# minfenli/refnerf-pl

Hardware: AMD Instinct MI355X
Metric: ray-samples/s (4096 rays x 128 samples x 2 levels, Ref-NeRF Blender, eval forward) (higher is better)
Workload: dtype f16x2; 1 GPU; blender_refnerf.gin, 4096 rays x 128 samples, 2-level, Model.__call__ eval forward with compute_extras + full ray_history; rays_per_gpu=4096, total_rays=4096, samples_per_level=128, parallelism=ray-tile dp1, n_ranks_seen=1, hip_graph_replay=False

## Files before the change

### refnerf-pl_amd/csrc/refnerf_hip.hip

```cpp
#include <hip/hip_runtime.h>

#include <cmath>
#include <cstdio>
#include <cstring>
#include <cstdlib>
#include <mutex>
#include <utility>
#include <vector>

#include "refnerf_hip.h"
#include "refnerf_level_common.h"
#include "refnerf_level_f32.h"
#include "refnerf_level_bf16.h"
#include "refnerf_level_bwd_f32.h"
#include "refnerf_wgrad.h"
#include "refnerf_wgrad_bf16x3.h"
#include "refnerf_rays.h"
#include "refnerf_pack_common.h"
#include "refnerf_sq_host.h"
#include "refnerf_sq_layout.h"

namespace rn {


// ... 659 lines not shown
  if (R <= 0) return fail(REFNERF_EINVAL, "refnerf_level_forward: R must be positive%s");
  if (cfg->n_samples <= 1) return fail(REFNERF_EINVAL, "num_samples must be > 1%s");
  if (cfg->ray_shape != 0 && cfg->ray_shape != 1) return fail(REFNERF_EINVAL, "ray_shape must be 'cone' or 'cylinder'%s");
  if (cfg->n_in < 1 || cfg->n_in > 512) return fail(REFNERF_EINVAL, "n_in must be in [1,512]%s");
  if (cfg->precision != REFNERF_PREC_F32 && cfg->precision != REFNERF_PREC_BF16 && cfg->precision != REFNERF_PREC_F16 &&
      cfg->precision != REFNERF_PREC_F16X2)
    return fail(REFNERF_EINVAL, "unknown precision mode%s");
  if (cfg->raydist < REFNERF_RAYDIST_NONE || cfg->raydist > REFNERF_RAYDIST_SQUARE)
    return fail(REFNERF_EINVAL, "unknown raydist (REFNERF_RAYDIST_*)%s");
  if (cfg->dir_enc != REFNERF_DIRENC_IDE && cfg->dir_enc != REFNERF_DIRENC_POSENC)
    return fail(REFNERF_EINVAL, "unknown dir_enc (REFNERF_DIRENC_IDE / REFNERF_DIRENC_POSENC)%s");
  if (cfg->training && cfg->precision == REFNERF_PREC_F16)
    return fail(REFNERF_EUNSUPPORTED, "REFNERF_PREC_F16 is an inference mode (training levels: REFNERF_PREC_F32, REFNERF_PREC_F16X2 or REFNERF_PREC_BF16)%s");
  const bool gbasis = cfg->ipe_groups > 1;
  if (cfg->ipe_groups < 0 || cfg->ipe_groups > rn::IPE_MAX_GROUPS) return fail(REFNERF_EINVAL, "ipe_groups must be in [0,7]%s");
  if (gbasis && cfg->precision != REFNERF_PREC_F32 && cfg->precision != REFNERF_PREC_F16X2)
    return fail(REFNERF_EUNSUPPORTED, "a general IPE basis (ipe_groups > 1) runs with REFNERF_PREC_F32 or REFNERF_PREC_F16X2 (d_packed: the REFNERF_PREC_F32 image of refnerf_pack_weights_basis in both)%s");
  const bool train_bf = cfg->training && cfg->precision == REFNERF_PREC_BF16;
  if (!rays->d_origins || !rays->d_directions || !rays->d_viewdirs || !rays->d_radii || !rays->d_near || !rays->d_far)
    return fail(REFNERF_EINVAL, "refnerf_level_forward: null ray field%s");
  const int N = cfg->n_samples;
  const bool gb_split = gbasis && cfg->precision == REFNERF_PREC_F16X2;
  if (int irc = check_image(d_packed, cfg, "refnerf_level_forward")) return irc;
  const bool train_sq = cfg->training && cfg->precision == REFNERF_PREC_F16X2 && !gbasis;
  if (train_sq && !d_act)
    return fail(REFNERF_EINVAL, "a training level in REFNERF_PREC_F16X2 runs through refnerf_level_forward_train: its kernel keeps the ReLU sign words and "
                                "the bottleneck rows in the activation buffer (d_packed: the REFNERF_IMAGE_F16X2_TRAIN image)%s");
  if (cfg->wgrad_mode == REFNERF_WGRAD_F16 && !train_sq)
    return fail(REFNERF_EUNSUPPORTED, "wgrad_mode = REFNERF_WGRAD_F16 belongs to training levels in REFNERF_PREC_F16X2 on the built-in IPE basis%s");
  if (train_sq) return rnsq::forward(d_packed, cfg, rays, R, d_sdist_in, d_weights_in, out, d_act, (hipStream_t)stream);
  const bool split = cfg->precision == REFNERF_PREC_F16X2 && !gb_split;
  const bool bf = (cfg->precision == REFNERF_PREC_BF16 && !train_bf) || cfg->precision == REFNERF_PREC_F16 || split;
  int rpw = rays_per_wg(N, bf ? rn::BT : rn::T_TILE);
  bool ps_ring = false;
  if (bf && N <= rn::BF_PS_RING - rn::BT && (rpw * N) % rn::BT != 0) {
    int r = 1;
    while (r <= rn::BF_NW && (r * N) % rn::BT != 0) ++r;
    if (r <= rn::BF_NW && r * N > 640 && R / r >= 512) { rpw = r; ps_ring = true; }
  }
  auto lds_bytes = [&](int rays) -> size_t {
    const int np = bf ? rn::NPS_EVAL : rn::NPS_TRAIN, tile = bf ? rn::BT : rn::T_TILE;
    const int ps_rows = ps_ring ? rn::BF_PS_RING : rays * N;
    const size_t per_wg = sizeof(float) * (size_t)(2 * rays * (N + 1) + np * ps_rows + 3 * tile + 8 + 12 * rays);
    if (bf) return (size_t)rn::BF_RING_BYTES + rn::BF_X_BYTES + sizeof(float) * rn::HD_ROWS * rn::BT + per_wg;
    return sizeof(float) * (size_t)(rn::DIR_PAD * rn::T_TILE + rn::HD_ROWS * rn::T_TILE) + per_wg;
  };
  if (ps_ring && lds_bytes(rpw) + (size_t)rt().lds_pad > 160 * 1024) { ps_ring = false; rpw = rays_per_wg(N, rn::BT); }
  if (bf && !ps_ring) while (2 * rpw <= rn::BF_NW && 2 * rpw * N <= 640 && lds_bytes(2 * rpw) <= 160 * 1024 &&
                 R / (2 * rpw) >= 512)
    rpw *= 2;
  if (rpw * N > 640 && !ps_ring) return fail(REFNERF_EINVAL, "n_samples too large for the LDS budget (rays_per_wg*N must be <= 640)%s");
  size_t lds = lds_bytes(rpw);
  {
    const int nwmax = bf ? rn::BF_NW : 4;
    const int nw = rpw < nwmax ? rpw : nwmax;
    const size_t scratch = sizeof(float) * (size_t)nw * (3 * (cfg->n_in + 4) + N + 3);
    if (scratch > (bf ? (size_t)rn::BF_X_BYTES : sizeof(float) * rn::DIR_PAD * rn::T_TILE))
      return fail(REFNERF_EINVAL, "n_in / n_samples too large for the resampler scratch of this precision mode%s");
  }
  while (train_bf && rpw > 1 && (lds + 15) / 16 * 16 + rn::RING_BYTES > 160 * 1024) { rpw /= 2; lds = lds_bytes(rpw); }
  const size_t ring_off = (lds + 15) / 16 * 16;
  if (train_bf) lds = ring_off + rn::RING_BYTES;
  lds += (size_t)rt().lds_pad;
  if (lds > 160 * 1024) return fail(REFNERF_EINVAL, "n_samples too large for the 160 KiB LDS budget of this precision mode%s");
  LDS_ATTR_ONCE(lds_attr(rn::level_fwd_f32), lds_attr(rn::level_fwd_train_f32), lds_attr(rn::level_fwd_train_bf16c),
                lds_attr(rn::level_fwd_bf16), lds_attr(rn::level_fwd_f16), lds_attr(rn::level_fwd_bf16_ring), lds_attr(rn::level_fwd_f16_ring),
                lds_attr(rn::level_fwd_f16x2), lds_attr(rn::level_fwd_f16x2_ring), lds_attr(rn::level_fwd_f32_gb), lds_attr(rn::level_fwd_train_f32_gb), lds_attr(rn::level_fwd_f16x2c_gb));
  rn::LevelArgs a;
  a.packed = d_packed;
  a.cfg = *cfg;
  a.rays = *rays;
  a.R = R;
  a.rpw = rpw;
  a.sdist_in = d_sdist_in;
  a.weights_in = d_weights_in;
  a.out = *out;
  a.prof = nullptr;
  a.g_means = nullptr; a.g_covs = nullptr; a.cov_full = 0;
  a.act = d_act; a.act_pitch = act_pitch;
  a.ring_off = (int)ring_off;
  if (rt().prof) {
    int prc = prof_buffer(&a.prof);
    if (prc) return prc;
  }
  int grid = (R + rpw - 1) / rpw;
  hipStream_t st = (hipStream_t)stream;
  long tslot = -1;
  {
    int trc = timer_begin(st, &tslot);
    if (trc) return trc;
  }
  if (split && ps_ring) hipLaunchKernelGGL(rn::level_fwd_f16x2_ring, dim3(grid), dim3(rn::BF_NTHREADS), lds, st, a);
  else if (split) hipLaunchKernelGGL(rn::level_fwd_f16x2, dim3(grid), dim3(rn::BF_NTHREADS), lds, st, a);
  else if (bf && ps_ring && cfg->precision == REFNERF_PREC_F16) hipLaunchKernelGGL(rn::level_fwd_f16_ring, dim3(grid), dim3(rn::BF_NTHREADS), lds, st, a);
  else if (bf && ps_ring) hipLaunchKernelGGL(rn::level_fwd_bf16_ring, dim3(grid), dim3(rn::BF_NTHREADS), lds, st, a);
  else if (bf && cfg->precision == REFNERF_PREC_F16) hipLaunchKernelGGL(rn::level_fwd_f16, dim3(grid), dim3(rn::BF_NTHREADS), lds, st, a);
  else if (bf) hipLaunchKernelGGL(rn::level_fwd_bf16, dim3(grid), dim3(rn::BF_NTHREADS), lds, st, a);
  else if (train_bf) hipLaunchKernelGGL(rn::level_fwd_train_bf16c, dim3(grid), dim3(rn::NTHREADS), lds, st, a);
  else if (gb_split) hipLaunchKernelGGL(rn::level_fwd_f16x2c_gb, dim3(grid), dim3(rn::NTHREADS), lds, st, a);
  else if (cfg->training && gbasis) hipLaunchKernelGGL(rn::level_fwd_train_f32_gb, dim3(grid), dim3(rn::NTHREADS), lds, st, a);
  else if (cfg->training) hipLaunchKernelGGL(rn::level_fwd_train_f32, dim3(grid), dim3(rn::NTHREADS), lds, st, a);
  else if (gbasis) hipLaunchKernelGGL(rn::level_fwd_f32_gb, dim3(grid), dim3(rn::NTHREADS), lds, st, a);
  else hipLaunchKernelGGL(rn::level_fwd_f32, dim3(grid), dim3(rn::NTHREADS), lds, st, a);
  HIP_TRY(hipGetLastError());
  {
    int trc = timer_end(st, tslot);
    if (trc) return trc;
  }
  if (a.prof) {
    long long hbuf[8 * 32];
    HIP_TRY(hipMemcpy(hbuf, a.prof, sizeof(hbuf), hipMemcpyDeviceToHost));
    const int nw = bf ? 8 : 4;
    for (int w = 0; w < nw; ++w) {
      fprintf(stderr, "[prof] wave %d:", w);
      for (int sl = 1; sl <= 18; ++sl) fprintf(stderr, " %lld", hbuf[w * 32 + sl] ? hbuf[w * 32 + sl] - hbuf[w * 32] : -1LL);
      fprintf(stderr, "  | dma-wait %lld barrier-wait %lld", hbuf[w * 32 + 20], hbuf[w * 32 + 21]);
      if (hbuf[w * 32 + 23] > hbuf[w * 32 + 22])
        fprintf(stderr, " | clock %.0f MHz", 100.0 * (double)(hbuf[w * 32 + 15] - hbuf[w * 32]) / (double)(hbuf[w * 32 + 23] - hbuf[w * 32 + 22]));
      fprintf(stderr, "\n");
    }
  }
  return REFNERF_OK;
}

int refnerf_level_forward(const void *d_packed, const refnerf_level_cfg *cfg, const refnerf_rays *rays,
                          int32_t R, const float *d_sdist_in, const float *d_weights_in,
                          const refnerf_level_out *out, void *stream) {
  return level_forward_impl(d_packed, cfg, rays, R, d_sdist_in, d_weights_in, out, nullptr, 0, stream);
}

int refnerf_level_forward_train(const void *d_packed, const refnerf_level_cfg *cfg, const refnerf_rays *rays,
                                int32_t R, const float *d_sdist_in, const float *d_weights_in,
                                const refnerf_level_out *out, void *d_activations, size_t activations_bytes,
                                void *stream) {
  if (!cfg || !d_activations) return fail(REFNERF_EINVAL, "refnerf_level_forward_train: null pointer%s");
  if (!cfg->training) return fail(REFNERF_EINVAL, "refnerf_level_forward_train: cfg->training must be 1%s");
  if (R <= 0 || cfg->n_samples <= 1) return fail(REFNERF_EINVAL, "refnerf_level_forward_train: bad R / num_samples%s");
  const BwdPlan plan = bwd_plan(R, cfg->n_samples, cfg->ipe_groups);
  if (activations_bytes < plan.act_bytes)
    return fail(REFNERF_EINVAL, "refnerf_level_forward_train: activation buffer too small (see refnerf_activation_workspace_bytes)%s");
  return level_forward_impl(d_packed, cfg, rays, R, d_sdist_in, d_weights_in, out, (float *)d_activations, plan.pitch, stream);
}

static int pixels_to_rays_impl(const char *fn, const int32_t *d_pix_x, const int32_t *d_pix_y, const float *d_pixtocams,
                               int32_t pixtocam_per_ray, const float *d_camtoworlds, int32_t camtoworld_per_ray,
                               const float *d_pixtocam_ndc, int32_t n, float *d_origins, float *d_directions, float *d_viewdirs,
                               float *d_radii, float *d_imageplane, const refnerf_lens_distortion *dist, void *stream) {
  if (!d_pix_x || !d_pix_y || !d_pixtocams || !d_camtoworlds || !d_origins || !d_directions || !d_viewdirs || !d_radii)
    return fail(REFNERF_EINVAL, "%s: null pointer", fn);
  if (n <= 0) return fail(REFNERF_EINVAL, "%s: n must be positive", fn);
  rn::RayGenArgs a{};
  a.pix_x = d_pix_x; a.pix_y = d_pix_y;
  a.pixtocams = d_pixtocams; a.camtoworlds = d_camtoworlds; a.pixtocam_ndc = d_pixtocam_ndc;
  a.p2c_stride = pixtocam_per_ray ? 9 : 0;
  a.c2w_stride = camtoworld_per_ray ? 12 : 0;
  a.n = n;
  a.origins = d_origins; a.directions = d_directions; a.viewdirs = d_viewdirs; a.radii = d_radii; a.imageplane = d_imageplane;
  if (dist) {
    a.dist = {dist->k1, dist->k2, dist->k3, dist->k4, dist->p1, dist->p2, dist->eps, dist->max_iterations};
    hipLaunchKernelGGL(rn::pixels_to_rays_kernel<true>, dim3((n + 255) / 256), dim3(256), 0, (hipStream_t)stream, a);
  } else {
    hipLaunchKernelGGL(rn::pixels_to_rays_kernel<false>, dim3((n + 255) / 256), dim3(256), 0, (hipStream_t)stream, a);
  }
  HIP_TRY(hipGetLastError());
  return REFNERF_OK;
}

int refnerf_pixels_to_rays(const int32_t *d_pix_x, const int32_t *d_pix_y, const float *d_pixtocams, int32_t pixtocam_per_ray,
                           const float *d_camtoworlds, int32_t camtoworld_per_ray, const float *d_pixtocam_ndc, int32_t n,
                           float *d_origins, float *d_directions, float *d_viewdirs, float *d_radii, float *d_imageplane,
                           void *stream) {
  return pixels_to_rays_impl("refnerf_pixels_to_rays", d_pix_x, d_pix_y, d_pixtocams, pixtocam_per_ray, d_camtoworlds,
                             camtoworld_per_ray, d_pixtocam_ndc, n, d_origins, d_directions, d_viewdirs, d_radii, d_imageplane,
                             nullptr, stream);
}

int refnerf_pixels_to_rays_distorted(const int32_t *d_pix_x, const int32_t *d_pix_y, const float *d_pixtocams,
                                     int32_t pixtocam_per_ray, const float *d_camtoworlds, int32_t camtoworld_per_ray,
                                     const float *d_pixtocam_ndc, int32_t n, float *d_origins, float *d_directions,
                                     float *d_viewdirs, float *d_radii, float *d_imageplane,
                                     const refnerf_lens_distortion *distortion, void *stream) {
  if (!distortion) return fail(REFNERF_EINVAL, "refnerf_pixels_to_rays_distorted: null distortion%s");
  const double c[7] = {distortion->k1, distortion->k2, distortion->k3, distortion->k4, distortion->p1, distortion->p2,
                       distortion->eps};
  for (double v : c)
    if (!std::isfinite(v)) return fail(REFNERF_EINVAL, "refnerf_pixels_to_rays_distorted: non-finite distortion parameter%s");
  if (distortion->max_iterations < 0 || distortion->max_iterations > REFNERF_MAX_UNDISTORT_ITERATIONS)
    return fail(REFNERF_EINVAL, "refnerf_pixels_to_rays_distorted: max_iterations must be in [0, 64]%s");
  return pixels_to_rays_impl("refnerf_pixels_to_rays_distorted", d_pix_x, d_pix_y, d_pixtocams, pixtocam_per_ray,
                             d_camtoworlds, camtoworld_per_ray, d_pixtocam_ndc, n, d_origins, d_directions, d_viewdirs,
                             d_radii, d_imageplane, distortion, stream);
}

int refnerf_mlp_forward(const void *d_packed, const refnerf_level_cfg *cfg, const float *d_means, const float *d_covs,
                        int32_t cov_is_full, const float *d_viewdirs, int32_t R, int32_t N, const refnerf_level_out *out,
                        void *stream) {
  if (!d_packed || !cfg || !d_means || !d_covs || !d_viewdirs || !out)
    return fail(REFNERF_EINVAL, "refnerf_mlp_forward: null pointer%s");
// ... 344 lines not shown
```

### refnerf-pl_amd/csrc/refnerf_level_bf16.h

```cpp
#pragma once
#include <type_traits>

#include "refnerf_level_common.h"

namespace rn {

typedef short v2s __attribute__((ext_vector_type(2)));

struct MmBf16 {
  typedef __bf16 t;
  typedef t v8 __attribute__((ext_vector_type(8)));
  typedef t v2 __attribute__((ext_vector_type(2)));
  static __device__ __forceinline__ v16f mfma(v8 a, v8 b, v16f c) { return __builtin_amdgcn_mfma_f32_32x32x16_bf16(a, b, c, 0, 0, 0); }
};
struct MmF16 {
  typedef _Float16 t;
  typedef t v8 __attribute__((ext_vector_type(8)));
  typedef t v2 __attribute__((ext_vector_type(2)));
  static __device__ __forceinline__ v16f mfma(v8 a, v8 b, v16f c) { return __builtin_amdgcn_mfma_f32_32x32x16_f16(a, b, c, 0, 0, 0); }
};
template <typename MM>
__device__ __forceinline__ unsigned cvt_pk_mm(float lo, float hi) {
  typename MM::v2 r = __builtin_convertvector((v2f){lo, hi}, typename MM::v2);
  return __builtin_bit_cast(unsigned, r);
// ... 555 lines not shown
    };
    if constexpr (LAYER0) sq_chunk<SQ_X, true, true>(p, fr, in, acc, prev, hook);
    else {
      sq_chunk<SQ_A, true, false>(p, fr, in, acc, prev, hook);
      sq_chunk<SQ_B, false, true>(p, fr, in, acc, prev);
      if (skip) sq_chunk<SQ_X, false, true>(p, fr, in, acc, prev);
    }
  }
#pragma unroll
  for (int q = 0; q < 4; ++q) sq_epi_piece(accs[0], q, out[14], out[15]);
  __builtin_amdgcn_sched_barrier(0);
}
__device__ __forceinline__ void sq_bias_now(const Pipe &p, SqAcc &acc) {
  if (!REFNERF_SQ_PREBIAS) return;
  const v4f *bp = reinterpret_cast<const v4f *>(p.wbuf + p.cur_off + (p.lane >> 4) * 16);
  acc.t0 = bp[0];
  acc.t1 = bp[4];
}

template <typename MM, int KIND0, int REAL0>
__device__ __forceinline__ void dir_layer(Pipe &p, typename MM::v8 (&a)[AF], int second, const v4uu (&in)[16], const v4uu (&bn)[8], v4uu (&out)[16]) {
#pragma unroll
  for (int ob = 0; ob < 8; ++ob) {
    v16f acc;
    bf_chunk<MM, KIND0, REAL0, true, true>(p, a, in, bn, acc);
    if constexpr (KIND0 == BF_REG) {
      if (second == 2) bf_chunk<MM, BF_BNLDS, BF_DIR_REAL_KS, false, true>(p, a, in, bn, acc);
    }
    pack_acc<MM, true>(acc, out[2 * ob], out[2 * ob + 1]);
    __builtin_amdgcn_sched_barrier(0);
  }
}

template <bool RINGPS = false>
__device__ __forceinline__ void level_fwd_split(const LevelArgs &A) {
  typedef MmF16 MM;
  constexpr int PSM = RINGPS ? BF_PS_RING - 1 : 0;
  typedef typename MM::v8 v8mm;
  typedef typename MM::t mm_t;
  extern __shared__ __attribute__((aligned(16))) float smem[];
  const refnerf_level_cfg &cfg = A.cfg;
  const int N = cfg.n_samples;
  const int tid = threadIdx.x, lane = tid & 63;
  const int wave = __builtin_amdgcn_readfirstlane(tid >> 6);
  const int rpw = A.rpw;
  const int ray0 = blockIdx.x * rpw;
  const int n_tot = rpw * N;
  const int n_pass = (n_tot + BT - 1) / BT;

  char *WB = reinterpret_cast<char *>(smem);
  char *Xb = WB + BF_RING_BYTES;
  float *HD = reinterpret_cast<float *>(Xb + BF_X_BYTES);
  float *TD = HD + HD_ROWS * BT;
  float *XP = TD + rpw * (N + 1);
  float *PS = XP + rpw * (N + 1);
  float *PX = PS + (RINGPS ? BF_PS_RING : n_tot) * NPS_EVAL;
  float *NRM = PX + 3 * BT;
  const float *RY = NRM + 8;

  const int h = lane >> 5, n = lane & 31;
  const int col = wave * 32 + n;

  Pipe p;
  p.src = reinterpret_cast<const char *>(A.packed) + wave * 3072 + lane * 16;
  p.src_end = nullptr;
  p.wbuf = WB;
  p.xp = Xb + (h * BT + col) * 16;
  p.xps = Xb + ((lane >> 4) * BT + wave * 16 + (lane & 15)) * 16;
  p.seq = 0;
  p.cur_off = 0; p.nxt_off = BF_CHUNK_BYTES; p.nx2_off = 2 * BF_CHUNK_BYTES; p.fil_off = (REFNERF_RING_SLOTS - 1) * BF_CHUNK_BYTES;
  p.dma_left = n_pass * SPPACKED.chunks_per_pass;
  p.lane = lane; p.wave = wave; p.h = h;
  p.t_vm = 0; p.t_bar = 0;
  RN_STAMPW(A, 0);
#ifdef REFNERF_PROF_WAITS
  if (A.prof && blockIdx.x == (gridDim.x >> 1) && lane == 0) A.prof[wave * 32 + 22] = (long long)__builtin_amdgcn_s_memrealtime();
#endif
  issue_chunk<true>(p, p.cur_off);
  issue_chunk<true>(p, p.nxt_off);
#if REFNERF_RING_SLOTS == 4
  issue_chunk<true>(p, p.nx2_off);
#endif

  resample_phase<BF_NW, true>(A, reinterpret_cast<float *>(Xb), TD, NRM, ray0, wave, lane);
#pragma clang loop unroll(disable)
  for (int rl = wave; rl < rpw; rl += BF_NW) {
    const int ray = ray0 + rl;
    if (ray >= A.R) break;
    float *RYw = NRM + 8 + rl * 12;
    if (lane < 10) {
      const float val = lane < 3 ? A.rays.d_origins[(size_t)ray * 3 + lane]
                      : lane < 6 ? A.rays.d_directions[(size_t)ray * 3 + lane - 3]
                      : lane < 9 ? A.rays.d_viewdirs[(size_t)ray * 3 + lane - 6] : A.rays.d_radii[ray];
      RYw[lane] = val;
      const float dx = __shfl(val, 3, 64), dy = __shfl(val, 4, 64), dz = __shfl(val, 5, 64);
      if (lane == 0) NRM[rl] = sqrtf((dx * dx + dy * dy) + dz * dz);
    }
  }
  RN_STAMPW(A, 1);
  asm volatile("s_waitcnt vmcnt(0)" ::: "memory");
  __syncthreads();
  RN_STAMPW(A, 2);

#ifndef REFNERF_BF_NOPRIO
  if (wave >= BF_NW / 2) __builtin_amdgcn_s_setprio(1);
#endif
  v4uu R0[16], R1[16];
  sq_v8 ar[SQ_NF];
#pragma unroll
  for (int d = 0; d < SQ_NF; ++d) ar[d] = lds_frag<MM>(WB + 1024 + lane * 16 + d * 1024);

  for (int pass0 = 0; pass0 < n_tot; pass0 += BT) {
    int lane_v = lane;
    asm volatile("" : "+v"(lane_v));
    auto locate = [&](int &g, int &rl, bool &valid) {
      int col_l = col, pass_l = pass0;
      asm volatile("" : "+v"(col_l), "+s"(pass_l));
      g = pass_l + col_l;
      rl = g / N;
      valid = (g < n_tot) && (ray0 + rl < A.R);
    };
    auto pass_epilogue = [&]() {
      if constexpr (RINGPS) {
        __syncthreads();
        const int end = (pass0 + BT < n_tot) ? pass0 + BT : n_tot;
        int td_o = (int)(TD - smem), xp_o = (int)(XP - smem), ps_o = (int)(PS - smem), nrm_o = (int)(NRM - smem), lane_e = lane, pass_e = pass0;
        int ntot_e = n_tot, ray0_e = ray0, wave_e = wave;
        asm volatile("" : "+s"(td_o), "+s"(xp_o), "+s"(ps_o), "+s"(nrm_o), "+v"(lane_e), "+s"(pass_e), "+s"(ntot_e), "+s"(ray0_e), "+s"(wave_e));
        composite_phase<BF_NW, false, NPS_EVAL, PSM>(A, smem + td_o, smem + xp_o, smem + ps_o, ntot_e, ray0_e, wave_e, lane_e, nullptr, smem + nrm_o,
                                                     pass_e / N, end / N);
      }
    };
    {
      const int g0 = pass0 + wave * 32;
      if (g0 >= n_tot || ray0 + g0 / N >= A.R) { idle_pass<true>(p); pass_epilogue(); continue; }
    }
    auto load_heads = [&](SampleHeads &sh) {
      int g, rl; bool valid;
      locate(g, rl, valid);
      int ci = col, ro = (valid ? rl : 0) * 12;
      asm volatile("" : "+v"(ci), "+v"(ro));
      float v[3], gp[3], raw_dif[3], raw_tint[3];
#pragma unroll
      for (int i = 0; i < 3; ++i) {
        v[i] = RY[ro + 6 + i];
        gp[i] = HD[(1 + i) * BT + ci];
        raw_dif[i] = HD[(5 + i) * BT + ci];
        raw_tint[i] = HD[(8 + i) * BT + ci];
      }
      sample_heads<false>(cfg, HD[0 * BT + ci], gp, HD[4 * BT + ci], raw_dif, raw_tint, v, sh);
    };

    v4uu bn0[4];
    auto heads = [&](auto RUN, v4uu (&bn)[8]) {
      constexpr int run = decltype(RUN)::value;
      SqAcc ha[2];
      sq_bias_now(p, ha[1]);
#pragma unroll
      for (int ob = 0; ob < 5; ++ob) {
        SqAcc &acc = ha[(ob + 1) & 1];
        if (ob < 4) {
          sq_chunk<SQ_BN, true, true>(p, ar, R1, acc, ha[ob & 1]);
#pragma unroll
          for (int e = 0; e < 4; ++e) {
            const unsigned pk = e == 0 ? pk_f16(acc.t0[0], acc.t0[1]) : (e == 1 ? pk_f16(acc.t0[2], acc.t0[3])
                              : (e == 2 ? pk_f16(acc.t1[0], acc.t1[1]) : pk_f16(acc.t1[2], acc.t1[3])));
            if (run == 0) bn0[ob][e] = pk;
            else {
              const v2uu r = __builtin_amdgcn_permlane16_swap(bn0[ob][e], pk, false, false);
              bn[2 * ob][e] = r[0];
              bn[2 * ob + 1][e] = r[1];
            }
          }
        } else {
          sq_chunk<SQ_SC, true, false>(p, ar, R1, acc, ha[ob & 1]);
          const int bq = lane_v >> 4;
          int csl = wave * 32 + 16 * run + (lane_v & 15) + 4 * bq * BT;
          asm volatile("" : "+v"(csl));
#pragma unroll
          for (int i = 0; i < 4; ++i)
            if (4 * bq + i < HD_ROWS) HD[i * BT + csl] = acc.t0[i];
        }
      }
      wave_sync();
    };
    typedef std::integral_constant<int, 0> Run0;
    typedef std::integral_constant<int, 1> Run1;

#pragma unroll 1
    for (int phase = 0; phase < 2; ++phase) {
#pragma unroll
      for (int e = 0; e < 16; ++e) { R0[e] = (v4uu){0, 0, 0, 0}; R1[e] = (v4uu){0, 0, 0, 0}; }
      {
      const int i16 = lane_v & 15, part = lane_v >> 4;
      const int hb = part >> 1, qq = part & 1;
      const int cs = wave * 32 + 16 * phase + i16;
      const int gs = pass0 + cs;
      const int rls = gs / N, sis = gs - rls * N;
      const bool vs = (gs < n_tot) && (ray0 + rls < A.R);
      float o[3], d[3];
      const float *ry = RY + (vs ? rls : 0) * 12;
#pragma unroll
      for (int i = 0; i < 3; ++i) { o[i] = ry[i]; d[i] = ry[3 + i]; }
      const float radius = ry[9];
      const float *td = TD + (vs ? rls : 0) * (N + 1);
      const float t0 = td[vs ? sis : 0], t1 = td[vs ? sis + 1 : 1];
      float lm[3], lv[3];
      cast_sample(o, d, radius, t0, t1, cfg.ray_shape, lm, lv);
      if (cfg.disable_integration) { lv[0] = 0.0f; lv[1] = 0.0f; lv[2] = 0.0f; }
      char *xw = Xb + (wave * 16 + i16) * 16;
      RN_STAMPW(A, 17);
#pragma clang loop unroll(disable)
      for (int t = 0; t < 12; ++t) {
        unsigned whi, wlo;
        {
          float f[2];
#pragma unroll
          for (int u = 0; u < 2; ++u) {
            const int kk = 2 * t + u;
            const int jj = kk / 3, b3 = kk - 3 * jj;
            const float m = b3 == 0 ? lm[0] : (b3 == 1 ? lm[1] : lm[2]);
            const float v = b3 == 0 ? lv[0] : (b3 == 1 ? lv[1] : lv[2]);
            f[u] = ipe_feature_split(m, v, 8 * qq + jj, hb);
          }
          split_pair_f16(f[0], f[1], whi, wlo);
        }
        char *dst = xw + (6 * hb + 3 * qq + (t >> 2)) * BT * 16 + (t & 3) * 4;
        *reinterpret_cast<unsigned *>(dst) = whi;
        *reinterpret_cast<unsigned *>(dst + (BT / 2) * 16) = wlo;
      }
      }
      RN_STAMPW(A, 18);
      wave_sync();
      RN_STAMPW(A, 3 + phase * 4);
      if (phase == 0) {
#pragma unroll
        for (int d = AF; d < SQ_NF; ++d) ar[d] = lds_frag<MM>(p.wbuf + p.cur_off + 1024 + lane_v * 16 + d * 1024);
      }
      SqAcc accs[2];
      sq_bias_now(p, accs[1]);
      sq_layer<true>(p, ar, accs, false, R0, R0);
      RN_STAMPW(A, 4 + phase * 4);
#pragma unroll 1
      for (int it = 0; it < 4; ++it) {
        sq_layer<false>(p, ar, accs, it == 2, R0, R1);
        if (it < 3) sq_layer<false>(p, ar, accs, false, R1, R0);
      }
      RN_STAMPW(A, 5 + phase * 4);
      if (phase == 0) {
        v4uu none[8];
        heads(Run0(), none);
        RN_STAMPW(A, 6);
      }
    }
    v4uu bn[8];
    heads(Run1(), bn);
    RN_STAMPW(A, 10);
#pragma unroll
    for (int e = 0; e < 16; ++e) { R0[e] = (v4uu){0, 0, 0, 0}; R1[e] = (v4uu){0, 0, 0, 0}; }
    {
    const int h4 = RINGPS ? (fresh_lane() >> 5) : h;
    char *xs = Xb + col * 16;
    {
      SampleHeads sh;
      load_heads(sh);
      float ide[40];
#pragma unroll
      for (int q = 36; q < 40; ++q) ide[q] = 0.0f;
      if (cfg.dir_enc == REFNERF_DIRENC_POSENC) posenc_eval<false, true>(sh.refd[0], sh.refd[1], sh.refd[2], h4, [&](int q, float val) { ide[q] = val; });
      else ide_eval<false>(sh.refd[0], sh.refd[1], sh.refd[2], sh.rough, h4, [&](int q, float val) { ide[q] = val; });
      if (h4 == 0) ide[36] = sh.dot;
#pragma unroll
      for (int q = 0; q < 5; ++q) {
        v8mm pk;
#pragma unroll
        for (int e = 0; e < 8; ++e) pk[e] = (mm_t)ide[q * 8 + e];
        *reinterpret_cast<v8mm *>(xs + (5 * h4 + q) * BT * 16) = pk;
      }
    }
    wave_sync();
    RN_STAMPW(A, 11);
    v8mm (&ad)[AF] = reinterpret_cast<v8mm (&)[AF]>(ar);
    dir_layer<MM, BF_BNLDS, BF_DIR_REAL_KS>(p, ad, 0, R0, bn, R0);
    RN_STAMPW(A, 12);
#pragma unroll 1
    for (int it = 0; it < 4; ++it) {
      dir_layer<MM, BF_REG, 0>(p, ad, (it == 2) ? 2 : 0, R0, bn, R1);
      if (it < 3) dir_layer<MM, BF_REG, 0>(p, ad, 0, R1, bn, R0);
    }
    RN_STAMPW(A, 13);
    v16f acc;
    bf_chunk<MM, BF_REG, 0, true, true>(p, ad, R1, bn, acc);
    float raw_rgb[3];
    const int lane6 = RINGPS ? fresh_lane() : lane;
    const int n6 = RINGPS ? (lane6 & 31) : n, h6 = RINGPS ? (lane6 >> 5) : h;
#pragma unroll
    for (int i = 0; i < 3; ++i) raw_rgb[i] = __shfl(acc[i], n6, 64);
    int g_w, rl_w; bool valid;
    locate(g_w, rl_w, valid);
    int lane_w = lane6, pass_w = pass0;
    asm volatile("" : "+v"(lane_w), "+s"(pass_w));
    if (valid && h6 == 0) {
      SampleHeads sh;
      load_heads(sh);
      colour_store<false, NPS_EVAL, PSM, true, RINGPS>(A, sh, raw_rgb, PS, PX, n_tot, g_w, RINGPS ? wave * 32 + n6 : col);
    }
    wave_sync();
    history_flush<NPS_EVAL, PSM>(A, PS, PX, n_tot, pass_w + wave * 32, wave * 32, (size_t)ray0 * N + pass_w + wave * 32, lane_w);
    RN_STAMPW(A, 14);
    }
    __builtin_amdgcn_wave_barrier();
    pass_epilogue();
  }
  asm volatile("s_waitcnt vmcnt(0)" ::: "memory");
  __syncthreads();
  RN_STAMPW(A, 15);
#ifdef REFNERF_PROF_WAITS
  if (A.prof && blockIdx.x == (gridDim.x >> 1) && lane == 0) {
    A.prof[wave * 32 + 20] = p.t_vm; A.prof[wave * 32 + 21] = p.t_bar;
    A.prof[wave * 32 + 23] = (long long)__builtin_amdgcn_s_memrealtime();
  }
#endif
  if constexpr (!RINGPS) composite_phase<BF_NW, false, NPS_EVAL>(A, TD, XP, PS, n_tot, ray0, wave, lane, reinterpret_cast<float *>(WB), NRM);
  RN_STAMPW(A, 16);
}

#ifndef REFNERF_SECONDARY_TU
__global__ __launch_bounds__(BF_NTHREADS) void level_fwd_f16x2(const LevelArgs A) { level_fwd_split<false>(A); }
__global__ __launch_bounds__(BF_NTHREADS) void level_fwd_f16x2_ring(const LevelArgs A) { level_fwd_split<true>(A); }
#endif

__device__ __forceinline__ int ipe_col_of_kprime(int kp) { return kp; }

}
```

### refnerf-pl_amd/csrc/refnerf_level_common.h

```cpp
#pragma once
#include <hip/hip_runtime.h>

#include "refnerf_hip.h"
#include "refnerf_device_math.h"
#include "refnerf_layout.h"

namespace rn {

typedef float v16f __attribute__((ext_vector_type(16)));
typedef float v4f __attribute__((ext_vector_type(4)));
typedef unsigned int v4u __attribute__((ext_vector_type(4)));

constexpr int NTHREADS = 256;

typedef __bf16 v8bf __attribute__((ext_vector_type(8)));
typedef unsigned v4uu __attribute__((ext_vector_type(4)));
typedef __bf16 v2bf __attribute__((ext_vector_type(2)));
typedef float v2f __attribute__((ext_vector_type(2)));
__device__ __forceinline__ unsigned cvt_pk_bf16(float lo, float hi) {
  v2bf r = __builtin_convertvector((v2f){lo, hi}, v2bf);
  return __builtin_bit_cast(unsigned, r);
}

constexpr int HD_ROWS = 12;
constexpr int NPS_EVAL = 17, NPS_TRAIN = 21;
enum { PS_DENSITY = 0, PS_RGB = 1, PS_DIF = 4, PS_SPC = 7, PS_NPRED = 10, PS_TINT = 13, PS_ROUGH = 16, PS_NORMALS = 17 };

struct LevelArgs {
  const void *packed;
  refnerf_level_cfg cfg;
  refnerf_rays rays;
  int R;
  int rpw;
  const float *sdist_in;
  const float *weights_in;
  refnerf_level_out out;
  long long *prof;
  const float *g_means;
  const float *g_covs;
  int cov_full;
  float *act;
  long long act_pitch;
  int ring_off;
};

#define RN_STAMP(A, slot) do { asm volatile("; RNMARK " #slot); if ((A).prof && blockIdx.x == (gridDim.x >> 1) && (threadIdx.x & 63) == 0) (A).prof[(threadIdx.x >> 6) * 32 + (slot)] = (long long)__builtin_readcyclecounter(); } while (0)

__device__ __forceinline__ int tile_hi(int col) {
  int hi = 128 * 128 + col;
  asm volatile("" : "+v"(hi));
  return hi;
}
__device__ __forceinline__ int tile_idx(int row, int col, int hi) { return row < 128 ? row * 128 + col : (row - 128) * 128 + hi; }

__device__ __forceinline__ void wave_sync() {
  __builtin_amdgcn_fence(__ATOMIC_SEQ_CST, "wavefront");
  __builtin_amdgcn_wave_barrier();
}

__device__ __forceinline__ float wave_sum(float v) {
#pragma unroll
  for (int o = 32; o > 0; o >>= 1) v += __shfl_xor(v, o, 64);
  return v;
}
__device__ __forceinline__ float wave_max(float v) {
#pragma unroll
  for (int o = 32; o > 0; o >>= 1) v = fmaxf(v, __shfl_xor(v, o, 64));
  return v;
}
constexpr int WSUM_PITCH = 65;
template <int K>
__device__ __forceinline__ void wave_sum_many(float (&v)[K], float *scr, int lane) {
#pragma unroll
  for (int k = 0; k < K; ++k) scr[k * WSUM_PITCH + lane] = v[k];
  __builtin_amdgcn_fence(__ATOMIC_SEQ_CST, "wavefront");
  __builtin_amdgcn_wave_barrier();
  float s = 0.0f;
  if (lane < K) {
    const float *col = scr + lane * WSUM_PITCH;
#pragma clang loop unroll(disable)
    for (int j = 0; j < 64; j += 4) s += (col[j] + col[j + 1]) + (col[j + 2] + col[j + 3]);
  }
#pragma unroll
  for (int k = 0; k < K; ++k) v[k] = __shfl(s, k, 64);
  __builtin_amdgcn_fence(__ATOMIC_SEQ_CST, "wavefront");
  __builtin_amdgcn_wave_barrier();
}

__device__ __forceinline__ float lane_value(float x, int l) {
  return __builtin_bit_cast(float, __builtin_amdgcn_readlane(__builtin_bit_cast(int, x), l));
}

__device__ __forceinline__ double wave_scan_incl(double v, int lane) {
#pragma unroll
  for (int o = 1; o < 64; o <<= 1) {
    double t = __shfl_up(v, o, 64);
    if (lane >= o) v += t;
  }
  return v;
}

template <bool EXACT = true>
__device__ __forceinline__ void sample_intervals_wave(const float *t_in, float *lg, float *cw, float *c, int M, int N,
                                      float smin, float smax, float *sd, int32_t *bin_idx_g, int lane) {
  float mx = -INFINITY;
  #pragma clang loop unroll(disable)
  for (int i = lane; i < M; i += 64) mx = fmaxf(mx, lg[i]);
  mx = wave_max(mx);
  #pragma clang loop unroll(disable)
  for (int i = lane; i < M; i += 64) lg[i] = rn_det_expf(lg[i] - mx);
  __builtin_amdgcn_fence(__ATOMIC_SEQ_CST, "wavefront");
  __builtin_amdgcn_wave_barrier();
  float sum = 0.0f;
  if (EXACT) {
    #pragma clang loop unroll(disable)
    for (int i0 = 0; i0 < M; i0 += 64) {
      const float x = (i0 + lane < M) ? lg[i0 + lane] : 0.0f;
#pragma unroll
      for (int l = 0; l < 64; ++l) sum += lane_value(x, l);
    }
  } else {
    #pragma clang loop unroll(disable)
    for (int i = lane; i < M; i += 64) sum += lg[i];
    sum = wave_sum(sum);
  }
  #pragma clang loop unroll(disable)
  for (int i = lane; i < M; i += 64) lg[i] = lg[i] / sum;
  __builtin_amdgcn_fence(__ATOMIC_SEQ_CST, "wavefront");
  __builtin_amdgcn_wave_barrier();
  if (EXACT) {
    double acc = 0.0;
    #pragma clang loop unroll(disable)
    for (int i0 = 0; i0 < M; i0 += 64) {
      const float x = (i0 + lane < M) ? lg[i0 + lane] : 0.0f;
      float mine = 0.0f;
#pragma unroll
      for (int l = 0; l < 64; ++l) {
        acc += (double)lane_value(x, l);
        mine = (lane == l) ? (float)acc : mine;
      }
      if (i0 + lane < M - 1) cw[i0 + lane + 1] = fminf(1.0f, mine);
    }
    if (lane == 0) { cw[0] = 0.0f; cw[M] = 1.0f; }
  } else {
    const int Cn = (M + 63) / 64, i0 = lane * Cn;
    double loc = 0.0;
    #pragma clang loop unroll(disable)
    for (int q = 0; q < Cn; ++q) if (i0 + q < M - 1) loc += (double)lg[i0 + q];
    double run = wave_scan_incl(loc, lane) - loc;
    #pragma clang loop unroll(disable)
    for (int q = 0; q < Cn; ++q) if (i0 + q < M - 1) { run += (double)lg[i0 + q]; cw[i0 + q + 1] = fminf(1.0f, (float)run); }
    if (lane == 0) { cw[0] = 0.0f; cw[M] = 1.0f; }
  }
  __builtin_amdgcn_fence(__ATOMIC_SEQ_CST, "wavefront");
  __builtin_amdgcn_wave_barrier();
  #pragma clang loop unroll(disable)
  for (int k = lane; k < N; k += 64) {
    float u = linspace_u(k, N);
    int lo = 0, hi = M;
    #pragma clang loop unroll(disable)
    while (hi - lo > 1) {
      int mid = (lo + hi) >> 1;
      if (u >= cw[mid]) lo = mid; else hi = mid;
    }
    float xp0 = cw[lo], xp1 = cw[lo + 1], fp0 = t_in[lo], fp1 = t_in[lo + 1];
    float q = (u - xp0) / (xp1 - xp0);
    if (q != q) q = 0.0f;
    float off = clip01(q);
    c[k] = fp0 + off * (fp1 - fp0);
    if (bin_idx_g) bin_idx_g[k] = lo;
  }
  __builtin_amdgcn_fence(__ATOMIC_SEQ_CST, "wavefront");
  __builtin_amdgcn_wave_barrier();
  #pragma clang loop unroll(disable)
  for (int k = lane; k <= N; k += 64) {
    float v;
    if (k == 0) v = fmaxf(smin, 2.0f * c[0] - (c[1] + c[0]) / 2.0f);
    else if (k == N) v = fminf(smax, 2.0f * c[N - 1] - (c[N - 1] + c[N - 2]) / 2.0f);
    else v = (c[k] + c[k - 1]) / 2.0f;
    sd[k] = v;
  }
  __builtin_amdgcn_fence(__ATOMIC_SEQ_CST, "wavefront");
  __builtin_amdgcn_wave_barrier();
}

__device__ __forceinline__ int fresh_lane() {
  int z = 0;
  asm volatile("" : "+v"(z));
  return (int)__builtin_amdgcn_mbcnt_hi(~0u, __builtin_amdgcn_mbcnt_lo(~0u, (unsigned)z));
}

__device__ __forceinline__ void st3(float *base, size_t idx, float a, float b, float c) {
  if (base) { base[idx * 3 + 0] = a; base[idx * 3 + 1] = b; base[idx * 3 + 2] = c; }
}


template <int NW = 4, bool EXACT = true>
__device__ __forceinline__ void resample_phase(const LevelArgs &A, float *scratch, float *TD, float *NRM, int ray0, int wave, int lane) {
  const refnerf_level_cfg &cfg = A.cfg;
  const int N = cfg.n_samples, M = cfg.n_in, rpw = A.rpw;
  const int Mp = (M + 4) & ~3, Np = (N + 3) & ~3;
  float *scr = scratch + wave * (3 * Mp + Np);
  float *t_in = scr, *lg = scr + Mp, *cw = scr + 2 * Mp, *c = scr + 3 * Mp;
  #pragma clang loop unroll(disable)
  for (int rl = wave; rl < rpw; rl += NW) {
    int ray = ray0 + rl;
    if (ray >= A.R) break;
    const float *tg = A.sdist_in + (size_t)ray * (M + 1);
    const float *wg = A.weights_in + (size_t)ray * M;
    #pragma clang loop unroll(disable)
    for (int i = lane; i <= M; i += 64) t_in[i] = tg[i];
    wave_sync();
    #pragma clang loop unroll(disable)
    for (int i = lane; i < M; i += 64)
      lg[i] = (t_in[i + 1] > t_in[i]) ? cfg.anneal * rn_det_logf(wg[i] + cfg.resample_padding) : -INFINITY;
    wave_sync();
    float *sd = TD + rl * (N + 1);
    sample_intervals_wave<EXACT>(t_in, lg, cw, c, M, N, cfg.s_near, cfg.s_far, sd,
                          A.out.d_bin_idx ? A.out.d_bin_idx + (size_t)ray * N : nullptr, lane);
    float nearv = A.rays.d_near[ray], farv = A.rays.d_far[ray];
    if (!EXACT) {
      float *RY = NRM + 8 + rl * 12;
      if (lane < 10) {
        const float val = lane < 3 ? A.rays.d_origins[(size_t)ray * 3 + lane]
                        : lane < 6 ? A.rays.d_directions[(size_t)ray * 3 + lane - 3]
                        : lane < 9 ? A.rays.d_viewdirs[(size_t)ray * 3 + lane - 6] : A.rays.d_radii[ray];
        RY[lane] = val;
        const float dx = __shfl(val, 3, 64), dy = __shfl(val, 4, 64), dz = __shfl(val, 5, 64);
        if (lane == 0) NRM[rl] = sqrtf((dx * dx + dy * dy) + dz * dz);
      }
    }
    #pragma clang loop unroll(disable)
    for (int k = lane; k <= N; k += 64) {
      float s = sd[k];
      if (A.out.d_sdist) A.out.d_sdist[(size_t)ray * (N + 1) + k] = s;
      sd[k] = s_to_t(s, nearv, farv, A.cfg.raydist);
    }
  }
}

struct SampleHeads {
  float density, rough, dot;
  float tint[3], raw_dif[3], npred[3], gp[3], refd[3];
  float normals[3] = {0.0f, 0.0f, 0.0f};
};
template <bool FAST = false>
__device__ __forceinline__ void sample_heads(const refnerf_level_cfg &cfg, float raw_density, const float gp[3],
                                             float raw_rough, const float raw_dif[3], const float raw_tint[3],
                                             const float v[3], SampleHeads &s) {
#pragma unroll
  for (int i = 0; i < 3; ++i) { s.gp[i] = gp[i]; s.raw_dif[i] = raw_dif[i]; s.tint[i] = sigmoid_m<FAST>(raw_tint[i]); }
  float n2 = fmaxf((gp[0] * gp[0] + gp[1] * gp[1]) + gp[2] * gp[2], EPS32);
  float nrm = sqrtf(n2);
#pragma unroll
  for (int i = 0; i < 3; ++i) s.npred[i] = -m_div<FAST>(gp[i], nrm);
  s.density = softplus_m<FAST>(raw_density + cfg.density_bias);
  s.rough = softplus_m<FAST>(raw_rough + cfg.roughness_bias);
  float w3[3] = {-v[0], -v[1], -v[2]};
  float dot = (s.npred[0] * w3[0] + s.npred[1] * w3[1]) + s.npred[2] * w3[2];
#pragma unroll
  for (int i = 0; i < 3; ++i) s.refd[i] = (2.0f * dot) * s.npred[i] - w3[i];
  s.dot = (s.npred[0] * v[0] + s.npred[1] * v[1]) + s.npred[2] * v[2];
}

template <int PSM>
__device__ __forceinline__ int ps_row(int g) { return PSM ? (g & PSM) : g; }

template <bool FAST = false, int NP = NPS_TRAIN, int PSM = 0, bool FAST_SRGB = FAST, bool PAD_HERE = false>
__device__ __forceinline__ void colour_store(const LevelArgs &A, const SampleHeads &s, const float raw_rgb[3],
                                             float *PS, float *PX, int n_tot, int g_sample, int gcol) {
  const int g = ps_row<PSM>(g_sample);
  const refnerf_level_cfg &cfg = A.cfg;
  float spec_lin[3], dif_lin[3], rgb[3], dif[3], spc[3];
#pragma unroll
  for (int i = 0; i < 3; ++i) {
    float sg = sigmoid_m<FAST>(cfg.rgb_premultiplier * raw_rgb[i] + cfg.rgb_bias);
    dif_lin[i] = sigmoid_m<FAST>(s.raw_dif[i] - LOG3_F);
    spec_lin[i] = s.tint[i] * sg;
    rgb[i] = spec_lin[i] + dif_lin[i];
  }
  if (cfg.srgb_mapping) {
    if (cfg.srgb_mapping_normalization) {
      float norm = fmaxf(fmaxf(fmaxf(rgb[0], rgb[1]), rgb[2]), 1.0f);
#pragma unroll
      for (int i = 0; i < 3; ++i) rgb[i] = m_div<FAST>(rgb[i], norm);
    }
#pragma unroll
    for (int i = 0; i < 3; ++i) {
      rgb[i] = clip01(linear_to_srgb<FAST_SRGB>(rgb[i]));
      dif[i] = clip01(linear_to_srgb<FAST_SRGB>(dif_lin[i]));
      spc[i] = clip01(linear_to_srgb<FAST_SRGB>(spec_lin[i]));
    }
  } else {
#pragma unroll
    for (int i = 0; i < 3; ++i) { dif[i] = dif_lin[i]; spc[i] = spec_lin[i]; }
  }
  float pad = cfg.rgb_padding;
  if (PAD_HERE) asm volatile("" : "+s"(pad));
  const float pad_scale = (float)(1.0 + 2.0 * (double)pad);
#pragma unroll
  for (int i = 0; i < 3; ++i) rgb[i] = rgb[i] * pad_scale - pad;
  PS[g * NP + PS_DENSITY] = s.density;
  PS[g * NP + PS_ROUGH] = s.rough;
#pragma unroll
  for (int i = 0; i < 3; ++i) {
    PS[g * NP + PS_RGB + i] = rgb[i];
    PS[g * NP + PS_DIF + i] = dif[i];
    PS[g * NP + PS_SPC + i] = spc[i];
    PS[g * NP + PS_NPRED + i] = s.npred[i];
    PS[g * NP + PS_TINT + i] = s.tint[i];
    if (NP > PS_NORMALS) PS[g * NP + PS_NORMALS + i] = s.normals[i];
    PX[gcol * 3 + i] = s.gp[i];
  }
}

#ifndef REFNERF_HIST_NT
#define REFNERF_HIST_NT 1
#endif
__device__ __forceinline__ void hist_store(float *p, float v) {
#if REFNERF_HIST_NT
  __builtin_nontemporal_store(v, p);
#else
  *p = v;
#endif
}

template <int NP = NPS_TRAIN, int PSM = 0>
__device__ __forceinline__ void history_flush(const LevelArgs &A, const float *PS, const float *PX, int n_tot, int gw0, int gcol0,
                                              size_t gs0, int lane) {
  const size_t total = (size_t)A.R * A.cfg.n_samples;
  auto vec3 = [&](float *dst, int slot) {
    if (!dst) return;
#pragma unroll
    for (int it = 0; it < 2; ++it) {
      const int f = lane + 64 * it;
      const int smp = f / 3, c = f - 3 * smp;
// ... 220 lines not shown
```

Baseline: 271.2 million ray-samples/s.

## Park sample heads in LDS, batch resample loads, cap VGPRs, add profiling stamps

```diff
diff --git a/refnerf-pl_amd/csrc/refnerf_hip.hip b/refnerf-pl_amd/csrc/refnerf_hip.hip
--- a/refnerf-pl_amd/csrc/refnerf_hip.hip
+++ b/refnerf-pl_amd/csrc/refnerf_hip.hip
@@ -765,6 +765,7 @@
   if (rt().prof) {
     int prc = prof_buffer(&a.prof);
     if (prc) return prc;
+    HIP_TRY(hipMemset(a.prof, 0, 8 * 32 * sizeof(long long)));
   }
   int grid = (R + rpw - 1) / rpw;
   hipStream_t st = (hipStream_t)stream;
@@ -797,6 +798,10 @@
     for (int w = 0; w < nw; ++w) {
       fprintf(stderr, "[prof] wave %d:", w);
       for (int sl = 1; sl <= 18; ++sl) fprintf(stderr, " %lld", hbuf[w * 32 + sl] ? hbuf[w * 32 + sl] - hbuf[w * 32] : -1LL);
+      if (split) {
+        fprintf(stderr, "  | parts");
+        for (int sl = 24; sl <= 31; ++sl) fprintf(stderr, " %lld", hbuf[w * 32 + sl] ? hbuf[w * 32 + sl] - hbuf[w * 32] : -1LL);
+      }
       fprintf(stderr, "  | dma-wait %lld barrier-wait %lld", hbuf[w * 32 + 20], hbuf[w * 32 + 21]);
       if (hbuf[w * 32 + 23] > hbuf[w * 32 + 22])
         fprintf(stderr, " | clock %.0f MHz", 100.0 * (double)(hbuf[w * 32 + 15] - hbuf[w * 32]) / (double)(hbuf[w * 32 + 23] - hbuf[w * 32 + 22]));
diff --git a/refnerf-pl_amd/csrc/refnerf_level_bf16.h b/refnerf-pl_amd/csrc/refnerf_level_bf16.h
--- a/refnerf-pl_amd/csrc/refnerf_level_bf16.h
+++ b/refnerf-pl_amd/csrc/refnerf_level_bf16.h
@@ -661,9 +661,8 @@
   issue_chunk<true>(p, p.nx2_off);
 #endif
 
-  resample_phase<BF_NW, true>(A, reinterpret_cast<float *>(Xb), TD, NRM, ray0, wave, lane);
 #pragma clang loop unroll(disable)
-  for (int rl = wave; rl < rpw; rl += BF_NW) {
+  for (int rl = (wave + BF_NW / 2) % BF_NW; rl < rpw; rl += BF_NW) {
     const int ray = ray0 + rl;
     if (ray >= A.R) break;
     float *RYw = NRM + 8 + rl * 12;
@@ -676,6 +675,7 @@
       if (lane == 0) NRM[rl] = sqrtf((dx * dx + dy * dy) + dz * dz);
     }
   }
+  resample_phase<BF_NW, true>(A, reinterpret_cast<float *>(Xb), TD, NRM, ray0, wave, lane, stamp_row(A, wave));
   RN_STAMPW(A, 1);
   asm volatile("s_waitcnt vmcnt(0)" ::: "memory");
   __syncthreads();
@@ -729,6 +729,29 @@
       }
       sample_heads<false>(cfg, HD[0 * BT + ci], gp, HD[4 * BT + ci], raw_dif, raw_tint, v, sh);
     };
+    auto park_heads = [&](const SampleHeads &sh) {
+      int ci = col;
+      asm volatile("" : "+v"(ci));
+      HD[0 * BT + ci] = sh.density;
+      HD[4 * BT + ci] = sh.rough;
+#pragma unroll
+      for (int i = 0; i < 3; ++i) HD[(8 + i) * BT + ci] = sh.tint[i];
+      HD[11 * BT + ci] = sh.nrm;
+    };
+    auto load_parked_heads = [&](SampleHeads &sh) {
+      int ci = col;
+      asm volatile("" : "+v"(ci));
+      sh.density = HD[0 * BT + ci];
+      sh.rough = HD[4 * BT + ci];
+      const float nrm = HD[11 * BT + ci];
+#pragma unroll
+      for (int i = 0; i < 3; ++i) {
+        sh.gp[i] = HD[(1 + i) * BT + ci];
+        sh.raw_dif[i] = HD[(5 + i) * BT + ci];
+        sh.tint[i] = HD[(8 + i) * BT + ci];
+        sh.npred[i] = -m_div<false>(sh.gp[i], nrm);
+      }
+    };
 
     v4uu bn0[4];
     auto heads = [&](auto RUN, v4uu (&bn)[8]) {
@@ -838,7 +861,7 @@
 #pragma unroll
     for (int e = 0; e < 16; ++e) { R0[e] = (v4uu){0, 0, 0, 0}; R1[e] = (v4uu){0, 0, 0, 0}; }
     {
-    const int h4 = RINGPS ? (fresh_lane() >> 5) : h;
+    const int h4 = fresh_lane() >> 5;
     char *xs = Xb + col * 16;
     {
       SampleHeads sh;
@@ -848,7 +871,7 @@
       for (int q = 36; q < 40; ++q) ide[q] = 0.0f;
       if (cfg.dir_enc == REFNERF_DIRENC_POSENC) posenc_eval<false, true>(sh.refd[0], sh.refd[1], sh.refd[2], h4, [&](int q, float val) { ide[q] = val; });
       else ide_eval<false>(sh.refd[0], sh.refd[1], sh.refd[2], sh.rough, h4, [&](int q, float val) { ide[q] = val; });
-      if (h4 == 0) ide[36] = sh.dot;
+      if (h4 == 0) { ide[36] = sh.dot; park_heads(sh); }
 #pragma unroll
       for (int q = 0; q < 5; ++q) {
         v8mm pk;
@@ -881,10 +904,11 @@
     asm volatile("" : "+v"(lane_w), "+s"(pass_w));
     if (valid && h6 == 0) {
       SampleHeads sh;
-      load_heads(sh);
+      load_parked_heads(sh);
       colour_store<false, NPS_EVAL, PSM, true, RINGPS>(A, sh, raw_rgb, PS, PX, n_tot, g_w, RINGPS ? wave * 32 + n6 : col);
     }
     wave_sync();
+    RN_STAMPW(A, 31);
     history_flush<NPS_EVAL, PSM>(A, PS, PX, n_tot, pass_w + wave * 32, wave * 32, (size_t)ray0 * N + pass_w + wave * 32, lane_w);
     RN_STAMPW(A, 14);
     }
@@ -905,7 +929,7 @@
 }
 
 #ifndef REFNERF_SECONDARY_TU
-__global__ __launch_bounds__(BF_NTHREADS) void level_fwd_f16x2(const LevelArgs A) { level_fwd_split<false>(A); }
+__global__ __launch_bounds__(BF_NTHREADS) __attribute__((amdgpu_num_vgpr(127))) void level_fwd_f16x2(const LevelArgs A) { level_fwd_split<false>(A); }
 __global__ __launch_bounds__(BF_NTHREADS) void level_fwd_f16x2_ring(const LevelArgs A) { level_fwd_split<true>(A); }
 #endif
 
diff --git a/refnerf-pl_amd/csrc/refnerf_level_common.h b/refnerf-pl_amd/csrc/refnerf_level_common.h
--- a/refnerf-pl_amd/csrc/refnerf_level_common.h
+++ b/refnerf-pl_amd/csrc/refnerf_level_common.h
@@ -46,6 +46,11 @@
 
 #define RN_STAMP(A, slot) do { asm volatile("; RNMARK " #slot); if ((A).prof && blockIdx.x == (gridDim.x >> 1) && (threadIdx.x & 63) == 0) (A).prof[(threadIdx.x >> 6) * 32 + (slot)] = (long long)__builtin_readcyclecounter(); } while (0)
 
+#define RN_STAMPP(pf, slot) do { if ((pf) && (threadIdx.x & 63) == 0) (pf)[slot] = (long long)__builtin_readcyclecounter(); } while (0)
+__device__ __forceinline__ long long *stamp_row(const LevelArgs &A, int wave) {
+  return (A.prof && blockIdx.x == (gridDim.x >> 1)) ? A.prof + wave * 32 : nullptr;
+}
+
 __device__ __forceinline__ int tile_hi(int col) {
   int hi = 128 * 128 + col;
   asm volatile("" : "+v"(hi));
@@ -102,7 +107,7 @@
 
 template <bool EXACT = true>
 __device__ __forceinline__ void sample_intervals_wave(const float *t_in, float *lg, float *cw, float *c, int M, int N,
-                                      float smin, float smax, float *sd, int32_t *bin_idx_g, int lane) {
+                                      float smin, float smax, float *sd, int32_t *bin_idx_g, int lane, long long *pf = nullptr) {
   float mx = -INFINITY;
   #pragma clang loop unroll(disable)
   for (int i = lane; i < M; i += 64) mx = fmaxf(mx, lg[i]);
@@ -128,6 +133,7 @@
   for (int i = lane; i < M; i += 64) lg[i] = lg[i] / sum;
   __builtin_amdgcn_fence(__ATOMIC_SEQ_CST, "wavefront");
   __builtin_amdgcn_wave_barrier();
+  RN_STAMPP(pf, 26);
   if (EXACT) {
     double acc = 0.0;
     #pragma clang loop unroll(disable)
@@ -154,6 +160,7 @@
   }
   __builtin_amdgcn_fence(__ATOMIC_SEQ_CST, "wavefront");
   __builtin_amdgcn_wave_barrier();
+  RN_STAMPP(pf, 27);
   #pragma clang loop unroll(disable)
   for (int k = lane; k < N; k += 64) {
     float u = linspace_u(k, N);
@@ -172,6 +179,7 @@
   }
   __builtin_amdgcn_fence(__ATOMIC_SEQ_CST, "wavefront");
   __builtin_amdgcn_wave_barrier();
+  RN_STAMPP(pf, 28);
   #pragma clang loop unroll(disable)
   for (int k = lane; k <= N; k += 64) {
     float v;
@@ -182,6 +190,7 @@
   }
   __builtin_amdgcn_fence(__ATOMIC_SEQ_CST, "wavefront");
   __builtin_amdgcn_wave_barrier();
+  RN_STAMPP(pf, 29);
 }
 
 __device__ __forceinline__ int fresh_lane() {
@@ -196,7 +205,8 @@
 
 
 template <int NW = 4, bool EXACT = true>
-__device__ __forceinline__ void resample_phase(const LevelArgs &A, float *scratch, float *TD, float *NRM, int ray0, int wave, int lane) {
+__device__ __forceinline__ void resample_phase(const LevelArgs &A, float *scratch, float *TD, float *NRM, int ray0, int wave, int lane,
+                                               long long *pf = nullptr) {
   const refnerf_level_cfg &cfg = A.cfg;
   const int N = cfg.n_samples, M = cfg.n_in, rpw = A.rpw;
   const int Mp = (M + 4) & ~3, Np = (N + 3) & ~3;
@@ -208,17 +218,27 @@
     if (ray >= A.R) break;
     const float *tg = A.sdist_in + (size_t)ray * (M + 1);
     const float *wg = A.weights_in + (size_t)ray * M;
-    #pragma clang loop unroll(disable)
-    for (int i = lane; i <= M; i += 64) t_in[i] = tg[i];
+    const float nearv = A.rays.d_near[ray], farv = A.rays.d_far[ray];
+    const float t_last = tg[M];
+    #pragma clang loop unroll(disable)
+    for (int i0 = 0; i0 < M; i0 += 128) {
+      const int ia = i0 + lane, ib = ia + 64;
+      const float ta = ia < M ? tg[ia] : 0.0f, tb = ib < M ? tg[ib] : 0.0f;
+      const float wa = ia < M ? wg[ia] : 0.0f, wb = ib < M ? wg[ib] : 0.0f;
+      if (ia < M) { t_in[ia] = ta; lg[ia] = wa; }
+      if (ib < M) { t_in[ib] = tb; lg[ib] = wb; }
+    }
+    if (lane == 0) t_in[M] = t_last;
     wave_sync();
+    RN_STAMPP(pf, 24);
     #pragma clang loop unroll(disable)
     for (int i = lane; i < M; i += 64)
-      lg[i] = (t_in[i + 1] > t_in[i]) ? cfg.anneal * rn_det_logf(wg[i] + cfg.resample_padding) : -INFINITY;
+      lg[i] = (t_in[i + 1] > t_in[i]) ? cfg.anneal * rn_det_logf(lg[i] + cfg.resample_padding) : -INFINITY;
     wave_sync();
+    RN_STAMPP(pf, 25);
     float *sd = TD + rl * (N + 1);
     sample_intervals_wave<EXACT>(t_in, lg, cw, c, M, N, cfg.s_near, cfg.s_far, sd,
-                          A.out.d_bin_idx ? A.out.d_bin_idx + (size_t)ray * N : nullptr, lane);
-    float nearv = A.rays.d_near[ray], farv = A.rays.d_far[ray];
+                          A.out.d_bin_idx ? A.out.d_bin_idx + (size_t)ray * N : nullptr, lane, pf);
     if (!EXACT) {
       float *RY = NRM + 8 + rl * 12;
       if (lane < 10) {
@@ -236,11 +256,13 @@
       if (A.out.d_sdist) A.out.d_sdist[(size_t)ray * (N + 1) + k] = s;
       sd[k] = s_to_t(s, nearv, farv, A.cfg.raydist);
     }
+    RN_STAMPP(pf, 30);
   }
 }
 
 struct SampleHeads {
   float density, rough, dot;
+  float nrm;
   float tint[3], raw_dif[3], npred[3], gp[3], refd[3];
   float normals[3] = {0.0f, 0.0f, 0.0f};
 };
@@ -252,6 +274,7 @@
   for (int i = 0; i < 3; ++i) { s.gp[i] = gp[i]; s.raw_dif[i] = raw_dif[i]; s.tint[i] = sigmoid_m<FAST>(raw_tint[i]); }
   float n2 = fmaxf((gp[0] * gp[0] + gp[1] * gp[1]) + gp[2] * gp[2], EPS32);
   float nrm = sqrtf(n2);
+  s.nrm = nrm;
 #pragma unroll
   for (int i = 0; i < 3; ++i) s.npred[i] = -m_div<FAST>(gp[i], nrm);
   s.density = softplus_m<FAST>(raw_density + cfg.density_bias);
```

Measured after the change: 272.2 million ray-samples/s (median of 6 runs). Within noise of the previous version (+0.4%).
